# knight46/Quantum_compute_DFT

Measured on AMD Instinct MI355X. Metric: grid_points_per_sec, higher is better.
Workload: dtype f64; 1 GPU; benzene_gga_def2svp: DFT_ComputeXC (GGA) nao=114 ngrid=143556 per GPU, synthetic AO/grid (SURVEY 8(d) recipe), inputs resident in HBM; functional=GGA, nao=114, nocc=21, ngrid_per_gpu=143556, entry_point=DFT_ComputeXC (the reference ABI: full density matrix)

## Files before the change

quantum_compute_dft_amd/csrc/xc_ws_kernels.hpp:

```cpp
#pragma once
#include <hip/hip_runtime.h>
#include "xc_kernels.hpp"

namespace qcdft {

#ifdef QCDFT_STAMPS
__device__ unsigned long long g_stamps[256 * 8 * 4];
#define QCDFT_T(var) unsigned long long var = __builtin_amdgcn_s_memtime()
#define QCDFT_ACC(slot, a, b) st_acc[slot] += (b) - (a)
#else
#define QCDFT_T(var)
#define QCDFT_ACC(slot, a, b)
#endif

constexpr int WS_ROWS = 16;
constexpr int WS_THREADS = 512;
constexpr int WS_RING = 4;
constexpr int WS_OT = 16;

template <int NT> struct WsCfg {
    static constexpr int NCOL = 16 * NT;
    static constexpr int JN = (NT + 1) / 2;
    static constexpr int LDA = NCOL + 2;
    static constexpr int LDX = ((NCOL + 31) / 32) * 32 + 16;
};

__device__ __forceinline__ unsigned ws_tile(unsigned ntile, unsigned b, unsigned s, unsigned nwg, int rev)
{
    const unsigned t = b + s * nwg;
    return rev ? ntile - 1u - t : t;
}

template <int NT, bool GRAD, bool VEC, bool SYM>
__global__ __launch_bounds__(WS_THREADS, 2) void k_vxc_ws(long ngrid, int nao,
                                                          const double *__restrict__ ao,
                                                          const double *__restrict__ gx,
                                                          const double *__restrict__ gy,
                                                          const double *__restrict__ gz,
                                                          const double *__restrict__ coef,
                                                          double *__restrict__ slabs, int rev)
{
    using C = WsCfg<NT>;
    constexpr int TILE = WS_ROWS * C::LDX;
    constexpr int NTW = (NT + 1) / 2;
    __shared__ double ring[2 * WS_RING * TILE];
    double *const Ps = ring, *const Qs = ring + WS_RING * TILE;

    const int tid = threadIdx.x;
    const int wave = __builtin_amdgcn_readfirstlane(tid >> 6);
    const long ntile = (ngrid + WS_ROWS - 1) / WS_ROWS;
    const long nloc = (ntile > (long)blockIdx.x) ? (ntile - blockIdx.x + gridDim.x - 1) / gridDim.x : 0;
    const long nstep = nloc + 2;

    if (wave < 4) {
        const int lane = tid & 63, li = lane & 15, lk = lane >> 4;
        const int wa = wave >> 1, wb = wave & 1;
        const int na = (NT - wa + 1) / 2, nb = (NT - wb + 1) / 2;
        d4 acc[NTW][NTW];
#pragma unroll
        for (int i = 0; i < NTW; ++i)
#pragma unroll
            for (int j = 0; j < NTW; ++j) acc[i][j] = (d4){0.0, 0.0, 0.0, 0.0};

#ifdef QCDFT_STAMPS
        unsigned long long st_acc[4] = {0, 0, 0, 0};
#endif
        const int fo = lk * C::LDX + li;
        double af[NTW], bf[NTW];
        auto load_frags = [&](int slot, int ks, double (&a_)[NTW], double (&b_)[NTW]) {
            const double *P = Ps + slot * TILE + fo + 4 * ks * C::LDX;
            const double *Q = Qs + slot * TILE + fo + 4 * ks * C::LDX;
#pragma unroll
            for (int i = 0; i < NTW; ++i) {
                a_[i] = Q[16 * min(wa + 2 * i, NT - 1)];
                b_[i] = P[16 * min(wb + 2 * i, NT - 1)];
            }
        };
#pragma unroll
        for (int i = 0; i < NTW; ++i) { af[i] = 0.0; bf[i] = 0.0; }
        for (long base = 0; base < nstep; base += WS_RING) {
#pragma unroll
            for (int u = 0; u < WS_RING; ++u) {
                const long step = base + u;
                QCDFT_T(ta);
                if (step >= 2 && step < nstep) {
                    if (step == 2) load_frags((u + 2) % WS_RING, 0, af, bf);
#pragma unroll
                    for (int ks = 0; ks < WS_ROWS / 4; ++ks) {
                        double an[NTW], bn[NTW];
                        if (ks + 1 < WS_ROWS / 4) load_frags((u + 2) % WS_RING, ks + 1, an, bn);
                        else                      load_frags((u + 3) % WS_RING, 0, an, bn);
#pragma unroll
                        for (int i = 0; i < NTW; ++i)
#pragma unroll
                            for (int j = 0; j < NTW; ++j)
                                if ((2 * i + 1 < NT || i < na) && (2 * j + 1 < NT || j < nb))
                                    acc[i][j] = mfma_f64(af[i], bf[j], acc[i][j]);
#pragma unroll
                        for (int i = 0; i < NTW; ++i) { af[i] = an[i]; bf[i] = bn[i]; }
                    }
                }
                QCDFT_T(tb);
                __syncthreads();
                QCDFT_T(tc);
                QCDFT_ACC(0, ta, tb);
                QCDFT_ACC(1, tb, tc);
            }
        }
#ifdef QCDFT_STAMPS
        if ((tid & 63) == 0) { g_stamps[(blockIdx.x * 8 + wave) * 4 + 0] = st_acc[0]; g_stamps[(blockIdx.x * 8 + wave) * 4 + 1] = st_acc[1]; }
#endif
        double *slab = slabs + (size_t)blockIdx.x * nao * nao;
        if (!SYM) {
#pragma unroll
            for (int i = 0; i < NTW; ++i)
#pragma unroll
                for (int j = 0; j < NTW; ++j) {
                    if (i >= na || j >= nb) continue;
                    const int b = 16 * (wb + 2 * j) + li;
#pragma unroll
                    for (int r = 0; r < 4; ++r) {
                        const int a = 16 * (wa + 2 * i) + lk + 4 * r;
                        if (a < nao && b < nao) slab[(size_t)a * nao + b] = acc[i][j][r];
                    }
                }
        } else {
            constexpr int LDM = C::NCOL + 1;
            static_assert(LDM * C::NCOL <= 2 * WS_RING * TILE, "M tile must fit in the ring");
            double *M = ring;
#pragma unroll
            for (int i = 0; i < NTW; ++i)
#pragma unroll
                for (int j = 0; j < NTW; ++j) {
                    if (i >= na || j >= nb) continue;
                    const int b = 16 * (wb + 2 * j) + li;
#pragma unroll
                    for (int r = 0; r < 4; ++r) M[(16 * (wa + 2 * i) + lk + 4 * r) * LDM + b] = acc[i][j][r];
                }
        }
    } else {
        __builtin_amdgcn_s_setprio(3);
        const int lt = tid - 256, row = lt >> 4, seg = lt & 15;
        const double *c0 = coef, *c1 = coef + (size_t)ngrid, *c2 = coef + 2 * (size_t)ngrid,
                     *c3 = coef + 3 * (size_t)ngrid;
        double p0[2][2 * C::JN], p1[2][2 * C::JN], p2[2][2 * C::JN], p3[2][2 * C::JN];
        double k0[2], k1[2], k2[2], k3[2];

        const long plane = ngrid * (long)nao;
        const unsigned voff = (unsigned)(row * nao + 2 * seg) * 8u, koff = (unsigned)row * 8u;
        const unsigned tile_b = (unsigned)(WS_ROWS * nao) * 8u, ktile_b = WS_ROWS * 8u;
        const unsigned plane_b = (unsigned)(plane * 8), coef_b = (unsigned)(ngrid * 8);
        const __amdgpu_buffer_rsrc_t r0 = plane_rsrc(ao, plane), r1 = plane_rsrc(GRAD ? gx : ao, plane),
                                     r2 = plane_rsrc(GRAD ? gy : ao, plane), r3 = plane_rsrc(GRAD ? gz : ao, plane),
                                     q0 = plane_rsrc(c0, ngrid), q1 = plane_rsrc(GRAD ? c1 : c0, ngrid),
                                     q2 = plane_rsrc(GRAD ? c2 : c0, ngrid), q3 = plane_rsrc(GRAD ? c3 : c0, ngrid);
        auto issue = [&](int set, unsigned s) {
            const bool live = s < (unsigned)nloc;
            const unsigned t = ws_tile((unsigned)ntile, blockIdx.x, s, gridDim.x, rev);
            const unsigned so = live ? t * tile_b : plane_b, ko = live ? t * ktile_b : coef_b;
            k0[set] = buf_load_f64(q0, koff, ko);
            if (GRAD) {
                k1[set] = buf_load_f64(q1, koff, ko);
                k2[set] = buf_load_f64(q2, koff, ko);
                k3[set] = buf_load_f64(q3, koff, ko);
            }
            buf_load_row<C::JN, VEC>(r0, voff, so, p0[set]);
            if (GRAD) {
                buf_load_row<C::JN, VEC>(r1, voff, so, p1[set]);
                buf_load_row<C::JN, VEC>(r2, voff, so, p2[set]);
                buf_load_row<C::JN, VEC>(r3, voff, so, p3[set]);
            }
        };
        issue(0, 0);
        __builtin_amdgcn_sched_barrier(0);
        issue(1, 1);
        __builtin_amdgcn_sched_barrier(0);
#ifdef QCDFT_STAMPS
        unsigned long long st_acc[4] = {0, 0, 0, 0};
#endif

        for (long base = 0; base < nstep; base += WS_RING) {
#pragma unroll
            for (int u = 0; u < WS_RING; ++u) {
                const long step = base + u;
                const int set = u & 1;
                QCDFT_T(ta);
#ifdef QCDFT_STAMPS
                asm volatile("s_waitcnt vmcnt(20)" ::: "memory");
#endif
                QCDFT_T(tw);
                {
                    double *P = Ps + u * TILE, *Q = Qs + u * TILE;
#pragma unroll
                    for (int j = 0; j < C::JN; ++j) {
                        const int c = 32 * j + 2 * seg;
                        if (c < C::NCOL) {
                            const double a0 = p0[set][2 * j], b0 = p0[set][2 * j + 1];
                            double qa = k0[set] * a0, qb = k0[set] * b0;
                            if (GRAD) {
                                qa += k1[set] * p1[set][2 * j] + k2[set] * p2[set][2 * j] + k3[set] * p3[set][2 * j];
                                qb += k1[set] * p1[set][2 * j + 1] + k2[set] * p2[set][2 * j + 1] + k3[set] * p3[set][2 * j + 1];
                            }
                            *reinterpret_cast<double2 *>(&Q[row * C::LDX + c]) = make_double2(qa, qb);
                            *reinterpret_cast<double2 *>(&P[row * C::LDX + c]) = make_double2(a0, b0);
                        }
                    }
                    QCDFT_T(tm);
                    issue(set, (unsigned)step + 2u);
                    QCDFT_ACC(3, tw, tm);
                }
                QCDFT_T(tb);
                __syncthreads();
                QCDFT_T(tc);
                QCDFT_ACC(0, ta, tw);
                QCDFT_ACC(1, tw, tb);
                QCDFT_ACC(2, tb, tc);
            }
        }
#ifdef QCDFT_STAMPS
        if ((tid & 63) == 0) { for (int q = 0; q < 4; ++q) g_stamps[(blockIdx.x * 8 + wave) * 4 + q] = st_acc[q]; }
#endif
    }
    if (SYM) {
        constexpr int LDM = C::NCOL + 1;
        const double *M = ring;
        __syncthreads();
        double *slab = slabs + (size_t)blockIdx.x * nao * nao;
        for (int e = tid; e < nao * nao; e += WS_THREADS) {
            const int a = e / nao, b = e - a * nao;
            slab[e] = M[a * LDM + b] + M[b * LDM + a];
        }
    }
}

template <int NT, bool GRAD, bool VEC>
__global__ __launch_bounds__(WS_THREADS, 2) void k_rho_ws(long ngrid, int nao,
                                                          const double *__restrict__ ao,
                                                          const double *__restrict__ gx,
                                                          const double *__restrict__ gy,
                                                          const double *__restrict__ gz,
                                                          const double *__restrict__ dm,
                                                          double *__restrict__ rho,
                                                          double *__restrict__ grad,
                                                          double *__restrict__ sigma, int rev)
{
    using C = WsCfg<NT>;
    constexpr int NKS = 4 * NT;
    constexpr int NTW = (NT + 3) / 4;
    constexpr int ATILE = WS_ROWS * C::LDA, XTILE = WS_ROWS * C::LDX;
    __shared__ double As[WS_RING * ATILE];
    __shared__ double Xs[2 * XTILE];
    __shared__ double Ob[(WS_OT + 1) * WS_ROWS * 4];

    const int tid = threadIdx.x;
    const int wave = __builtin_amdgcn_readfirstlane(tid >> 6);
    const long ntile = (ngrid + WS_ROWS - 1) / WS_ROWS;
    const long nloc = (ntile > (long)blockIdx.x) ? (ntile - blockIdx.x + gridDim.x - 1) / gridDim.x : 0;
    const long nstep = nloc + 2;

    if (wave < 4) {
        const int lane = tid & 63, li = lane & 15, lk = lane >> 4;
        const int nks = (nao + 3) >> 2;
        const bool two = NTW > 1 && wave + 4 < NT;
        double dreg[NTW][NKS];
#pragma unroll
        for (int i = 0; i < NTW; ++i) {
            const int tcol = min(wave + 4 * i, NT - 1);
            const int n = 16 * tcol + li;
#pragma unroll
            for (int ks = 0; ks < NKS; ++ks) {
                const int k = 4 * ks + lk;
                const bool in = k < nao && n < nao;
                const int kc = in ? k : 0, nc = in ? n : 0;
                const double v = 0.5 * (dm[(size_t)kc * nao + nc] + dm[(size_t)nc * nao + kc]);
                dreg[i][ks] = in ? v : 0.0;
            }
        }
        for (long base = 0; base < nstep; base += WS_RING) {
#pragma unroll
            for (int u = 0; u < WS_RING; ++u) {
                const long step = base + u;
                if (step >= 1 && step <= nloc && wave < NT) {
                    const double *ap = As + ((u + 3) % WS_RING) * ATILE + li * C::LDA + lk;
                    double *X = Xs + ((u + 1) & 1) * XTILE;
                    d4 acc[NTW];
#pragma unroll
                    for (int i = 0; i < NTW; ++i) acc[i] = (d4){0.0, 0.0, 0.0, 0.0};
#pragma unroll
                    for (int ks = 0; ks < NKS; ++ks) {
                        if (ks < NKS - 3 || ks < nks) {
                            const double a = ap[4 * ks];
                            acc[0] = mfma_f64(a, dreg[0][ks], acc[0]);
                            if (NTW > 1) {
                                if (two) acc[NTW - 1] = mfma_f64(a, dreg[NTW - 1][ks], acc[NTW - 1]);
                            }
                        }
                    }
#pragma unroll
                    for (int r = 0; r < 4; ++r) {
                        X[(lk + 4 * r) * C::LDX + 16 * wave + li] = acc[0][r];
                        if (NTW > 1) {
                            if (two) X[(lk + 4 * r) * C::LDX + 16 * (wave + 4) + li] = acc[NTW - 1][r];
                        }
                    }
                }
                __syncthreads();
            }
        }
    } else {
        __builtin_amdgcn_s_setprio(3);
        const int lt = tid - 256, row = lt >> 4, seg = lt & 15;
        double ph[2][2 * C::JN];
        double pgx[2][2 * C::JN], pgy[2][2 * C::JN], pgz[2][2 * C::JN];

        auto row_of = [&](long s) { return (long)ws_tile((unsigned)ntile, blockIdx.x, (unsigned)s, gridDim.x, rev) * WS_ROWS + row; };
        const long plane = ngrid * (long)nao;
        const unsigned voff = (unsigned)(row * nao + 2 * seg) * 8u;
        const unsigned tile_b = (unsigned)(WS_ROWS * nao) * 8u, plane_b = (unsigned)(plane * 8);
        const __amdgpu_buffer_rsrc_t r0 = plane_rsrc(ao, plane), r1 = plane_rsrc(GRAD ? gx : ao, plane),
                                     r2 = plane_rsrc(GRAD ? gy : ao, plane), r3 = plane_rsrc(GRAD ? gz : ao, plane);
        auto tile_off = [&](unsigned s) {
            return s < (unsigned)nloc ? ws_tile((unsigned)ntile, blockIdx.x, s, gridDim.x, rev) * tile_b : plane_b;
        };
        auto issue_ao = [&](int set, unsigned s) { buf_load_row<C::JN, VEC>(r0, voff, tile_off(s), ph[set]); };
        auto issue_grad = [&](int set, unsigned s) {
            const unsigned so = tile_off(s);
            buf_load_row<C::JN, VEC>(r1, voff, so, pgx[set]);
            buf_load_row<C::JN, VEC>(r2, voff, so, pgy[set]);
            buf_load_row<C::JN, VEC>(r3, voff, so, pgz[set]);
        };
        issue_ao(0, 0);
        __builtin_amdgcn_sched_barrier(0);
        if (GRAD) issue_grad(0, (unsigned)nloc);
        __builtin_amdgcn_sched_barrier(0);
        issue_ao(1, 1);
        __builtin_amdgcn_sched_barrier(0);
        if (GRAD) issue_grad(1, (unsigned)nloc);
        __builtin_amdgcn_sched_barrier(0);

        long flushed = 0;
        auto flush = [&](long j0, long j1) {
            const long j = j0 + (lt >> 4);
            const int r = lt & 15;
            if (j < j1 && j < nloc) {
                const long g = (long)ws_tile((unsigned)ntile, blockIdx.x, (unsigned)j, gridDim.x, rev) * WS_ROWS + r;
                if (g < ngrid) {
                    const double *o = Ob + ((j % (WS_OT + 1)) * WS_ROWS + r) * 4;
                    rho[g] = o[0];
                    if (GRAD) {
                        const double ax = o[1], ay = o[2], az = o[3];
                        grad[3 * g + 0] = ax;
                        grad[3 * g + 1] = ay;
                        grad[3 * g + 2] = az;
                        sigma[g] = ax * ax + ay * ay + az * az;
                    }
                }
            }
        };
        for (long base = 0; base < nstep; base += WS_RING) {
#pragma unroll
            for (int u = 0; u < WS_RING; ++u) {
                const long step = base + u;
                const int set = u & 1;
                {
                    double *A = As + u * ATILE;
#pragma unroll
                    for (int j = 0; j < C::JN; ++j) {
                        const int c = 32 * j + 2 * seg;
                        if (c < C::NCOL)
                            *reinterpret_cast<double2 *>(&A[row * C::LDA + c]) = make_double2(ph[set][2 * j], ph[set][2 * j + 1]);
                    }
                    issue_ao(set, (unsigned)step + 2u);
                }
                {
                    const bool in_range = step >= 2 && step - 2 < nloc;
                    const long g = row_of(in_range ? step - 2 : 0);
                    const bool row_ok = in_range && g < ngrid;
                    const double *A = As + ((u + 2) % WS_RING) * ATILE;
                    const double *X = Xs + (u & 1) * XTILE;
                    double s0 = 0.0, s1 = 0.0, s2 = 0.0, s3 = 0.0;
#pragma unroll
                    for (int j = 0; j < C::JN; ++j) {
                        const int c = 32 * j + 2 * seg;
                        if (c < C::NCOL) {
                            const double2 x = *reinterpret_cast<const double2 *>(&X[row * C::LDX + c]);
                            const double2 p = *reinterpret_cast<const double2 *>(&A[row * C::LDA + c]);
                            s0 += x.x * p.x + x.y * p.y;
                            if (GRAD) {
                                s1 += x.x * pgx[set][2 * j] + x.y * pgx[set][2 * j + 1];
                                s2 += x.x * pgy[set][2 * j] + x.y * pgy[set][2 * j + 1];
                                s3 += x.x * pgz[set][2 * j] + x.y * pgz[set][2 * j + 1];
                            }
                        }
                    }
                    s0 = row16_sum(s0);
                    if (GRAD) {
                        s1 = row16_sum(s1);
                        s2 = row16_sum(s2);
                        s3 = row16_sum(s3);
                    }
                    (void)row_ok;
                    if (seg == 0 && in_range) {
                        double *o = Ob + (((step - 2) % (WS_OT + 1)) * WS_ROWS + row) * 4;
                        o[0] = s0;
                        if (GRAD) { o[1] = 2.0 * s1; o[2] = 2.0 * s2; o[3] = 2.0 * s3; }
                    }
                }
                if (step - 2 - flushed == WS_OT) {
                    flush(flushed, step - 2);
                    flushed = step - 2;
                }
                if (GRAD) issue_grad(set, (unsigned)step);
                __syncthreads();
            }
        }
        flush(flushed, nloc);
    }
}

__global__ __launch_bounds__(256) void k_finish_exc(long npart, const double *__restrict__ partial,
                                                    double *__restrict__ exc_dev, double *exc_host)
{
    __shared__ double part[4];
    double x = 0.0;
    for (long i = threadIdx.x; i < npart; i += 256) x += partial[i];
    for (int m = 32; m >= 1; m >>= 1) x += __shfl_down(x, m, 64);
    if ((threadIdx.x & 63) == 0) part[threadIdx.x >> 6] = x;
    __syncthreads();
    if (threadIdx.x == 0) {
        const double e = (part[0] + part[1]) + (part[2] + part[3]);
        exc_dev[0] = e;
        if (exc_host) {
            *(volatile double *)exc_host = e;
            __threadfence_system();
        }
    }
}

__global__ void k_publish_exc(const double *__restrict__ exc_dev, double *exc_host)
{
    *(volatile double *)exc_host = exc_dev[0];
    __threadfence_system();
}

template <bool SYM, bool FIN = false>
__global__ __launch_bounds__(256) void k_reduce_slabs8(int nao, int nslab,
                                                       const double *__restrict__ slabs,
                                                       double *__restrict__ V,
                                                       long npart = 0, const double *__restrict__ partial = nullptr,
                                                       double *__restrict__ exc_dev = nullptr, double *exc_host = nullptr)
{
    __shared__ double part[256];
    const size_t n2 = (size_t)nao * nao;
    const int el = threadIdx.x & 31, grp = threadIdx.x >> 5;
    const size_t e = (size_t)blockIdx.x * 32 + el;
    double s = 0.0;
    if (e < n2) {
        const int a = (int)(e / nao), b = (int)(e - (size_t)a * nao);
        const size_t et = (size_t)b * nao + a;
        int k = grp;
        for (; k + 8 * 15 < nslab; k += 8 * 16) {
            double v[16];
#pragma unroll
            for (int q = 0; q < 16; ++q) {
                v[q] = slabs[(size_t)(k + 8 * q) * n2 + e];
                if (SYM) v[q] += slabs[(size_t)(k + 8 * q) * n2 + et];
            }
#pragma unroll
            for (int q = 0; q < 16; ++q) s += v[q];
        }
        for (; k < nslab; k += 8) {
            double v = slabs[(size_t)k * n2 + e];
            if (SYM) v += slabs[(size_t)k * n2 + et];
            s += v;
        }
    }
    part[threadIdx.x] = s;
    __syncthreads();
    if (grp == 0 && e < n2) {
        const double *p = &part[el];
        V[e] = ((p[0] + p[32]) + (p[64] + p[96])) + ((p[128] + p[160]) + (p[192] + p[224]));
    }
    if (FIN) {
        if (blockIdx.x == gridDim.x - 1) {
            __syncthreads();
            double x = 0.0;
            for (long i = threadIdx.x; i < npart; i += 256) x += partial[i];
            part[threadIdx.x] = x;
            __syncthreads();
            for (int m = 128; m >= 1; m >>= 1) {
                if ((int)threadIdx.x < m) part[threadIdx.x] += part[threadIdx.x + m];
                __syncthreads();
            }
            if (threadIdx.x == 0) {
                exc_dev[0] = part[0];
                if (exc_host) {
                    *(volatile double *)exc_host = part[0];
                    __threadfence_system();
                }
            }
        }
    }
}

__global__ __launch_bounds__(256) void k_symmetrize(int nao, const double *__restrict__ M,
                                                    double *__restrict__ V)
{
    __shared__ double A[32][33], B[32][33];
    const int nt = (nao + 31) / 32;
    int ti = 0, rem = blockIdx.x;
    while (rem >= nt - ti) { rem -= nt - ti; ++ti; }
    const int tj = ti + rem;
    const int tx = threadIdx.x & 31, ty = threadIdx.x >> 5;
    for (int r = ty; r < 32; r += 8) {
        const int a = 32 * ti + r, b = 32 * tj + tx;
        A[r][tx] = (a < nao && b < nao) ? M[(size_t)a * nao + b] : 0.0;
        const int a2 = 32 * tj + r, b2 = 32 * ti + tx;
        B[r][tx] = (a2 < nao && b2 < nao) ? M[(size_t)a2 * nao + b2] : 0.0;
    }
    __syncthreads();
    for (int r = ty; r < 32; r += 8) {
        const int a = 32 * ti + r, b = 32 * tj + tx;
        if (a < nao && b < nao) V[(size_t)a * nao + b] = A[r][tx] + B[tx][r];
        const int a2 = 32 * tj + r, b2 = 32 * ti + tx;
        if (ti != tj && a2 < nao && b2 < nao) V[(size_t)a2 * nao + b2] = A[tx][r] + B[r][tx];
    }
}

}
```

Baseline: 626.9 million grid-points/s.

## Offload row reductions to MFMA waves and strength-reduce tile offsets

Replaces the per-row 16-lane shuffle reductions in the load/contract waves with a store of partial sums to a new LDS buffer. The MFMA waves then reduce those sums one pipeline step later using an MFMA against a constant vector, which adds a third pipeline stage. Tile offsets now come from a running increment instead of recomputing ws_tile per load, and loop counters switch to unsigned. The goal is to take shuffle and index arithmetic off the latency-critical load waves, at the cost of extra LDS, an extra step of pipeline depth, and more complex ring-slot bookkeeping.

Measured after the change: 652.4 million grid-points/s (median of 6 runs). 4.1% higher.

```diff
diff --git a/quantum_compute_dft_amd/csrc/xc_ws_kernels.hpp b/quantum_compute_dft_amd/csrc/xc_ws_kernels.hpp
--- a/quantum_compute_dft_amd/csrc/xc_ws_kernels.hpp
+++ b/quantum_compute_dft_amd/csrc/xc_ws_kernels.hpp
@@ -248,15 +248,20 @@
     constexpr int NKS = 4 * NT;
     constexpr int NTW = (NT + 3) / 4;
     constexpr int ATILE = WS_ROWS * C::LDA, XTILE = WS_ROWS * C::LDX;
+    constexpr int NQ = GRAD ? 4 : 1;
+    constexpr int LDS_ = WS_ROWS + 2, SQ = 320, STILE = NQ * SQ;
+    static_assert(WS_ROWS * LDS_ <= SQ, "a partial-sum plane must fit its stride");
     __shared__ double As[WS_RING * ATILE];
     __shared__ double Xs[2 * XTILE];
+    __shared__ double Ss[2 * STILE];
     __shared__ double Ob[(WS_OT + 1) * WS_ROWS * 4];
 
     const int tid = threadIdx.x;
     const int wave = __builtin_amdgcn_readfirstlane(tid >> 6);
-    const long ntile = (ngrid + WS_ROWS - 1) / WS_ROWS;
-    const long nloc = (ntile > (long)blockIdx.x) ? (ntile - blockIdx.x + gridDim.x - 1) / gridDim.x : 0;
-    const long nstep = nloc + 2;
+    const unsigned ntile = (unsigned)((ngrid + WS_ROWS - 1) / WS_ROWS);
+    const unsigned nwg = gridDim.x, wg = blockIdx.x;
+    const unsigned nloc = ntile > wg ? (ntile - wg + nwg - 1) / nwg : 0u;
+    const unsigned nstep = nloc + 3;
 
     if (wave < 4) {
         const int lane = tid & 63, li = lane & 15, lk = lane >> 4;
@@ -276,10 +281,14 @@
                 dreg[i][ks] = in ? v : 0.0;
             }
         }
-        for (long base = 0; base < nstep; base += WS_RING) {
+        const double *sp = Ss + min(wave, NQ - 1) * SQ + li * LDS_ + lk;
+        const double ones = wave == 0 ? 1.0 : 2.0;
+        double *op = Ob + lk * 4 + wave;
+        unsigned oslot = 0;
+        for (unsigned base = 0; base < nstep; base += WS_RING) {
 #pragma unroll
             for (int u = 0; u < WS_RING; ++u) {
-                const long step = base + u;
+                const unsigned step = base + u;
                 if (step >= 1 && step <= nloc && wave < NT) {
                     const double *ap = As + ((u + 3) % WS_RING) * ATILE + li * C::LDA + lk;
                     double *X = Xs + ((u + 1) & 1) * XTILE;
@@ -304,6 +313,18 @@
                         }
                     }
                 }
+                if (step >= 3 && step - 3 < nloc && wave < NQ) {
+                    const double *S = sp + ((u + 1) & 1) * STILE;
+                    d4 t = (d4){0.0, 0.0, 0.0, 0.0};
+#pragma unroll
+                    for (int ks = 0; ks < WS_ROWS / 4; ++ks) t = mfma_f64(S[4 * ks], ones, t);
+                    if (li == 0) {
+                        double *o = op + oslot * (WS_ROWS * 4);
+#pragma unroll
+                        for (int r = 0; r < 4; ++r) o[16 * r] = t[r];
+                    }
+                    oslot = oslot == WS_OT ? 0u : oslot + 1u;
+                }
                 __syncthreads();
             }
         }
@@ -313,39 +334,44 @@
         double ph[2][2 * C::JN];
         double pgx[2][2 * C::JN], pgy[2][2 * C::JN], pgz[2][2 * C::JN];
 
-        auto row_of = [&](long s) { return (long)ws_tile((unsigned)ntile, blockIdx.x, (unsigned)s, gridDim.x, rev) * WS_ROWS + row; };
         const long plane = ngrid * (long)nao;
         const unsigned voff = (unsigned)(row * nao + 2 * seg) * 8u;
         const unsigned tile_b = (unsigned)(WS_ROWS * nao) * 8u, plane_b = (unsigned)(plane * 8);
         const __amdgpu_buffer_rsrc_t r0 = plane_rsrc(ao, plane), r1 = plane_rsrc(GRAD ? gx : ao, plane),
                                      r2 = plane_rsrc(GRAD ? gy : ao, plane), r3 = plane_rsrc(GRAD ? gz : ao, plane);
-        auto tile_off = [&](unsigned s) {
-            return s < (unsigned)nloc ? ws_tile((unsigned)ntile, blockIdx.x, s, gridDim.x, rev) * tile_b : plane_b;
+        unsigned o_run = (rev ? ntile - 1u - wg : wg) * tile_b, left = nloc;
+        const unsigned o_inc = rev ? 0u - nwg * tile_b : nwg * tile_b;
+        auto next_off = [&]() {
+            const unsigned o = left ? o_run : plane_b;
+            left = left ? left - 1u : 0u;
+            o_run += o_inc;
+            return o;
         };
-        auto issue_ao = [&](int set, unsigned s) { buf_load_row<C::JN, VEC>(r0, voff, tile_off(s), ph[set]); };
-        auto issue_grad = [&](int set, unsigned s) {
-            const unsigned so = tile_off(s);
+        auto issue_ao = [&](int set, unsigned so) { buf_load_row<C::JN, VEC>(r0, voff, so, ph[set]); };
+        auto issue_grad = [&](int set, unsigned so) {
             buf_load_row<C::JN, VEC>(r1, voff, so, pgx[set]);
             buf_load_row<C::JN, VEC>(r2, voff, so, pgy[set]);
             buf_load_row<C::JN, VEC>(r3, voff, so, pgz[set]);
         };
-        issue_ao(0, 0);
+        unsigned o_a = next_off(), o_b = next_off();
+        issue_ao(0, o_a);
         __builtin_amdgcn_sched_barrier(0);
-        if (GRAD) issue_grad(0, (unsigned)nloc);
+        if (GRAD) issue_grad(0, plane_b);
         __builtin_amdgcn_sched_barrier(0);
-        issue_ao(1, 1);
+        issue_ao(1, o_b);
         __builtin_amdgcn_sched_barrier(0);
-        if (GRAD) issue_grad(1, (unsigned)nloc);
+        if (GRAD) issue_grad(1, plane_b);
         __builtin_amdgcn_sched_barrier(0);
 
-        long flushed = 0;
-        auto flush = [&](long j0, long j1) {
-            const long j = j0 + (lt >> 4);
+        auto flush = [&](unsigned j0, unsigned slot0) {
+            const unsigned j = j0 + (unsigned)(lt >> 4);
             const int r = lt & 15;
-            if (j < j1 && j < nloc) {
-                const long g = (long)ws_tile((unsigned)ntile, blockIdx.x, (unsigned)j, gridDim.x, rev) * WS_ROWS + r;
+            if (j < nloc) {
+                const long g = (long)ws_tile(ntile, wg, j, nwg, rev) * WS_ROWS + r;
                 if (g < ngrid) {
-                    const double *o = Ob + ((j % (WS_OT + 1)) * WS_ROWS + r) * 4;
+                    unsigned slot = slot0 + (unsigned)(lt >> 4);
+                    slot = slot > (unsigned)WS_OT ? slot - (WS_OT + 1) : slot;
+                    const double *o = Ob + (slot * WS_ROWS + r) * 4;
                     rho[g] = o[0];
                     if (GRAD) {
                         const double ax = o[1], ay = o[2], az = o[3];
@@ -357,11 +383,13 @@
                 }
             }
         };
-        for (long base = 0; base < nstep; base += WS_RING) {
+        unsigned flushed = 0, fslot = 0, fcount = WS_OT + 3 + 1;
+        double *const sw = Ss + row * LDS_ + seg;
+        for (unsigned base = 0; base < nstep; base += WS_RING) {
 #pragma unroll
             for (int u = 0; u < WS_RING; ++u) {
-                const long step = base + u;
                 const int set = u & 1;
+                const unsigned o_c = next_off();
                 {
                     double *A = As + u * ATILE;
 #pragma unroll
@@ -370,12 +398,9 @@
                         if (c < C::NCOL)
                             *reinterpret_cast<double2 *>(&A[row * C::LDA + c]) = make_double2(ph[set][2 * j], ph[set][2 * j + 1]);
                     }
-                    issue_ao(set, (unsigned)step + 2u);
+                    issue_ao(set, o_c);
                 }
                 {
-                    const bool in_range = step >= 2 && step - 2 < nloc;
-                    const long g = row_of(in_range ? step - 2 : 0);
-                    const bool row_ok = in_range && g < ngrid;
                     const double *A = As + ((u + 2) % WS_RING) * ATILE;
                     const double *X = Xs + (u & 1) * XTILE;
                     double s0 = 0.0, s1 = 0.0, s2 = 0.0, s3 = 0.0;
@@ -385,36 +410,36 @@
                         if (c < C::NCOL) {
                             const double2 x = *reinterpret_cast<const double2 *>(&X[row * C::LDX + c]);
                             const double2 p = *reinterpret_cast<const double2 *>(&A[row * C::LDA + c]);
-                            s0 += x.x * p.x + x.y * p.y;
-                            if (GRAD) {
-                                s1 += x.x * pgx[set][2 * j] + x.y * pgx[set][2 * j + 1];
-                                s2 += x.x * pgy[set][2 * j] + x.y * pgy[set][2 * j + 1];
-                                s3 += x.x * pgz[set][2 * j] + x.y * pgz[set][2 * j + 1];
+                            const double t0 = x.x * p.x + x.y * p.y;
+                            const double t1 = x.x * pgx[set][2 * j] + x.y * pgx[set][2 * j + 1];
+                            const double t2 = x.x * pgy[set][2 * j] + x.y * pgy[set][2 * j + 1];
+                            const double t3 = x.x * pgz[set][2 * j] + x.y * pgz[set][2 * j + 1];
+                            if (j == 0) {
+                                s0 = t0;
+                                if (GRAD) { s1 = t1; s2 = t2; s3 = t3; }
+                            } else {
+                                s0 += t0;
+                                if (GRAD) { s1 += t1; s2 += t2; s3 += t3; }
                             }
                         }
                     }
-                    s0 = row16_sum(s0);
-                    if (GRAD) {
-                        s1 = row16_sum(s1);
-                        s2 = row16_sum(s2);
-                        s3 = row16_sum(s3);
-                    }
-                    (void)row_ok;
-                    if (seg == 0 && in_range) {
-                        double *o = Ob + (((step - 2) % (WS_OT + 1)) * WS_ROWS + row) * 4;
-                        o[0] = s0;
-                        if (GRAD) { o[1] = 2.0 * s1; o[2] = 2.0 * s2; o[3] = 2.0 * s3; }
-                    }
-                }
-                if (step - 2 - flushed == WS_OT) {
-                    flush(flushed, step - 2);
-                    flushed = step - 2;
-                }
-                if (GRAD) issue_grad(set, (unsigned)step);
+                    double *S = sw + (u & 1) * STILE;
+                    S[0] = s0;
+                    if (GRAD) { S[SQ] = s1; S[2 * SQ] = s2; S[3 * SQ] = s3; }
+                }
+                if (--fcount == 0) {
+                    flush(flushed, fslot);
+                    flushed += WS_OT;
+                    fslot = fslot == 0 ? (unsigned)WS_OT : fslot - 1u;
+                    fcount = WS_OT;
+                }
+                if (GRAD) issue_grad(set, o_a);
+                o_a = o_b;
+                o_b = o_c;
                 __syncthreads();
             }
         }
-        flush(flushed, nloc);
+        flush(flushed, fslot);
     }
 }
 
```
